# intel/oim

Hardware: AMD Instinct MI355X
Metric: 4KiB_randread_IOPS (higher is better)
Workload: dtype uint8

## Files before the change

### native/src/gpu.hip

```cpp

#include <hip/hip_runtime.h>
#include <pthread.h>
#include <sched.h>
#include <unistd.h>
#include <stdlib.h>

#include <algorithm>
#include <atomic>
#include <chrono>
#include <condition_variable>
#include <cstring>
#include <deque>
#include <functional>
#include <map>
#include <mutex>
#include <random>
#include <set>
#include <stdexcept>
#include <thread>
#include <utility>
#include <vector>

#include "gpu_internal.h"
#include "hipstore/engine.h"

namespace hipstore {


namespace {

constexpr uint32_t kTileBytes = 4096;
constexpr uint32_t kRingSlots = 1 << 16;
constexpr uint32_t kMaxBatchTiles = kRingSlots / 4;

struct BlockDesc {
  const uint8_t* src;
  uint8_t* dst;
  uint32_t bytes;
  uint32_t fill;
};
static_assert(sizeof(BlockDesc) == 24, "persistent engine reads 3 x u64");

__global__ __launch_bounds__(kWavesPerWg * 64) void k_copy_blocks(
    const BlockDesc* __restrict__ descs, uint32_t n) {
  __shared__ __attribute__((aligned(16))) uint8_t lds_raw[kWavesPerWg * kTileBytes];
  const uint32_t wave = threadIdx.x >> 6;
  const uint32_t lane = threadIdx.x & 63;
  const uint32_t idx = blockIdx.x * kWavesPerWg + wave;
  if (idx >= n) return;
  const BlockDesc d = descs[idx];
  float4* lds = reinterpret_cast<float4*>(lds_raw + wave * kTileBytes);
  const uint32_t n16 = d.bytes >> 4;
  if (d.src != nullptr) {
    const float4* __restrict__ src = reinterpret_cast<const float4*>(d.src);
#pragma unroll 4
    for (uint32_t i = lane; i < n16; i += 64) lds[i] = src[i];
  } else {
    const uint32_t b = d.fill & 0xFF;
    const uint32_t word = b | (b << 8) | (b << 16) | (b << 24);
    const float4 v = {__uint_as_float(word), __uint_as_float(word),
                      __uint_as_float(word), __uint_as_float(word)};
    for (uint32_t i = lane; i < n16; i += 64) lds[i] = v;
  }
  float4* __restrict__ dst = reinterpret_cast<float4*>(d.dst);
#pragma unroll 4
  for (uint32_t i = lane; i < n16; i += 64) dst[i] = lds[i];
}


__device__ __forceinline__ unsigned long long wave_bcast_u64(
    unsigned long long v) {
  int lo = __shfl(static_cast<int>(v & 0xFFFFFFFFu), 0);
  int hi = __shfl(static_cast<int>(v >> 32), 0);
  return (static_cast<unsigned long long>(static_cast<uint32_t>(hi)) << 32) |
         static_cast<uint32_t>(lo);
}

__device__ __forceinline__ unsigned long long claim_bounded(
    unsigned long long* counter, unsigned long long c,
    unsigned long long kt, uint32_t lane) {
  while (c < kt) {
    unsigned long long witnessed = 0;
    if (lane == 0) {
      witnessed = atomicCAS(counter, c, c + 1);
    }
    witnessed = wave_bcast_u64(witnessed);
    if (witnessed == c) return c;
    c = witnessed;
  }
  return ~0ull;
}

struct PersistentCtl {
  const BlockDesc* sq;
  volatile unsigned long long* sq_tail;
  volatile unsigned long long* cq;
  volatile uint32_t* stop;
  unsigned long long* claim_counter;
  unsigned long long* known_tail;
  uint32_t* exit_flag;
  uint32_t ring_mask;
  uint32_t idle_spins;
};

__global__ __launch_bounds__(64) void k_persistent_copy(PersistentCtl ctl) {
  __shared__ __attribute__((aligned(16))) uint8_t lds_raw[kTileBytes];
  const uint32_t lane = threadIdx.x & 63;
  float4* lds = reinterpret_cast<float4*>(lds_raw);

  if (blockIdx.x == 0) {
    if (lane != 0) return;
    unsigned long long known = __hip_atomic_load(
        ctl.known_tail, __ATOMIC_RELAXED, __HIP_MEMORY_SCOPE_AGENT);
    uint32_t spins = 0;
    while (true) {
      unsigned long long tail = __hip_atomic_load(
          const_cast<const unsigned long long*>(ctl.sq_tail),
          __ATOMIC_ACQUIRE, __HIP_MEMORY_SCOPE_SYSTEM);
      if (tail > known) {
        known = tail;
        __hip_atomic_store(ctl.known_tail, known, __ATOMIC_RELEASE,
                           __HIP_MEMORY_SCOPE_AGENT);
        spins = 0;
      }
      if (__hip_atomic_load(const_cast<const uint32_t*>(ctl.stop),
                            __ATOMIC_RELAXED,
                            __HIP_MEMORY_SCOPE_SYSTEM) != 0 ||
          ++spins > ctl.idle_spins) {
        __hip_atomic_store(ctl.exit_flag, 1u, __ATOMIC_RELEASE,
                           __HIP_MEMORY_SCOPE_AGENT);
        return;
      }
      __builtin_amdgcn_s_sleep(8);
    }
  }

  while (true) {
    const unsigned long long kt = __hip_atomic_load(
        ctl.known_tail, __ATOMIC_RELAXED, __HIP_MEMORY_SCOPE_AGENT);
    const unsigned long long c = __hip_atomic_load(
        ctl.claim_counter, __ATOMIC_RELAXED, __HIP_MEMORY_SCOPE_AGENT);
    const unsigned long long claim =
        claim_bounded(ctl.claim_counter, c, kt, lane);
    if (claim == ~0ull) {
      if (__hip_atomic_load(ctl.exit_flag, __ATOMIC_RELAXED,
                            __HIP_MEMORY_SCOPE_AGENT) != 0) {
        return;
      }
      __builtin_amdgcn_s_sleep(16);
      continue;
    }
    const volatile unsigned long long* vd =
        reinterpret_cast<const volatile unsigned long long*>(
            &ctl.sq[claim & ctl.ring_mask]);
    const unsigned long long w0 = vd[0];
    const unsigned long long w1 = vd[1];
    const unsigned long long w2 = vd[2];
    BlockDesc d;
    d.src = reinterpret_cast<const uint8_t*>(w0);
    d.dst = reinterpret_cast<uint8_t*>(w1);
    d.bytes = static_cast<uint32_t>(w2 & 0xFFFFFFFFu);
    d.fill = static_cast<uint32_t>(w2 >> 32);
    const uint32_t n8 = d.bytes >> 3;
    unsigned long long* lds64 = reinterpret_cast<unsigned long long*>(lds);
    if (d.src != nullptr) {
      const unsigned long long* __restrict__ src =
          reinterpret_cast<const unsigned long long*>(d.src);
#pragma unroll 4
      for (uint32_t i = lane; i < n8; i += 64) {
        lds64[i] = __hip_atomic_load(src + i, __ATOMIC_RELAXED,
                                     __HIP_MEMORY_SCOPE_AGENT);
      }
    } else {
      const uint32_t b = d.fill & 0xFF;
      const uint32_t word = b | (b << 8) | (b << 16) | (b << 24);
      const unsigned long long v =
          word | (static_cast<unsigned long long>(word) << 32);
      for (uint32_t i = lane; i < n8; i += 64) lds64[i] = v;
    }
    unsigned long long* __restrict__ dst =
        reinterpret_cast<unsigned long long*>(d.dst);
#pragma unroll 4
    for (uint32_t i = lane; i < n8; i += 64) dst[i] = lds64[i];
    if (lane == 0) {
      __hip_atomic_store(&ctl.cq[claim & ctl.ring_mask], claim + 1,
                         __ATOMIC_RELEASE, __HIP_MEMORY_SCOPE_SYSTEM);
    }
  }
}

__global__ void k_init_ctl(unsigned long long* dst, unsigned long long a,
                           unsigned long long b, unsigned long long c) {
  if (threadIdx.x == 0) {
    dst[0] = a;
    dst[1] = b;
    dst[2] = c;
  }
}

std::atomic<uint64_t> g_pers_launches{0};
std::atomic<uint64_t> g_pers_relaunches{0};
std::atomic<uint64_t> g_pers_stall_queries{0};


struct SharedSlot {
  const BlockDesc* sq;
  volatile unsigned long long* sq_tail;
  volatile unsigned long long* cq;
  unsigned long long claim;
  unsigned long long known_tail;
  unsigned long long ring_mask_active;
};
static_assert(sizeof(SharedSlot) == 48, "8-byte atom layout");

constexpr uint32_t kSharedSlots = 64;

struct SharedCtl {
  SharedSlot* slots;
  volatile uint32_t* stop;
  uint32_t* exit_flag;
  uint32_t idle_spins;
};

__device__ __forceinline__ unsigned long long slot_ld(
    SharedSlot* slot, int word) {
  return __hip_atomic_load(
      reinterpret_cast<unsigned long long*>(slot) + word, __ATOMIC_RELAXED,
      __HIP_MEMORY_SCOPE_AGENT);
}

__device__ __forceinline__ void slot_st(SharedSlot* slot, int word,
                                        unsigned long long value) {
  __hip_atomic_store(reinterpret_cast<unsigned long long*>(slot) + word,
                     value, __ATOMIC_RELEASE, __HIP_MEMORY_SCOPE_AGENT);
}

__global__ __launch_bounds__(64) void k_shared_service(SharedCtl ctl) {
  __shared__ __attribute__((aligned(16))) uint8_t lds_raw[kTileBytes];
  const uint32_t lane = threadIdx.x & 63;
  float4* lds = reinterpret_cast<float4*>(lds_raw);

  if (blockIdx.x == 0) {
    SharedSlot* slot = &ctl.slots[lane];
    unsigned long long known = 0;
    uint32_t spins = 0;
    while (true) {
      bool advanced = false;
      if (slot_ld(slot, 5) >> 32) {
        volatile unsigned long long* tail_ptr =
            reinterpret_cast<volatile unsigned long long*>(slot_ld(slot, 1));
        const unsigned long long tail = __hip_atomic_load(
            const_cast<const unsigned long long*>(tail_ptr),
            __ATOMIC_ACQUIRE, __HIP_MEMORY_SCOPE_SYSTEM);
        if (tail > known) {
          known = tail;
          slot_st(slot, 4, known);
          advanced = true;
        }
      } else {
        known = 0;
      }
      const bool stop_now =
          lane == 0 &&
          __hip_atomic_load(const_cast<const uint32_t*>(ctl.stop),
                            __ATOMIC_RELAXED,
                            __HIP_MEMORY_SCOPE_SYSTEM) != 0;
      if (__any(advanced)) spins = 0;
      if (__any(stop_now) || ++spins > ctl.idle_spins) {
        if (lane == 0) {
          __hip_atomic_store(ctl.exit_flag, 1u, __ATOMIC_RELEASE,
                             __HIP_MEMORY_SCOPE_AGENT);
        }
        return;
      }
      __builtin_amdgcn_s_sleep(8);
    }
  }

  const uint32_t start = blockIdx.x;
  while (true) {
    bool progress = false;
    for (uint32_t i = 0; i < kSharedSlots; ++i) {
      SharedSlot* slot = &ctl.slots[(start + i) % kSharedSlots];
      const unsigned long long ma = slot_ld(slot, 5);
      if (!(ma >> 32)) continue;
      const uint32_t ring_mask = static_cast<uint32_t>(ma);
      const unsigned long long kt = slot_ld(slot, 4);
      const unsigned long long c = slot_ld(slot, 3);
      const unsigned long long claim =
          claim_bounded(&slot->claim, c, kt, lane);
      if (claim == ~0ull) continue;
      const BlockDesc* sq = reinterpret_cast<const BlockDesc*>(slot_ld(slot, 0));
      const volatile unsigned long long* vd =
          reinterpret_cast<const volatile unsigned long long*>(
              &sq[claim & ring_mask]);
      const unsigned long long w0 = vd[0];
      const unsigned long long w1 = vd[1];
      const unsigned long long w2 = vd[2];
      const uint8_t* src = reinterpret_cast<const uint8_t*>(w0);
      uint8_t* dst = reinterpret_cast<uint8_t*>(w1);
      const uint32_t bytes = static_cast<uint32_t>(w2 & 0xFFFFFFFFu);
      const uint32_t n8 = bytes >> 3;
      unsigned long long* lds64 =
          reinterpret_cast<unsigned long long*>(lds);
      if (src != nullptr) {
        const unsigned long long* __restrict__ s8 =
            reinterpret_cast<const unsigned long long*>(src);
#pragma unroll 4
        for (uint32_t k = lane; k < n8; k += 64) {
          lds64[k] = __hip_atomic_load(s8 + k, __ATOMIC_RELAXED,
                                       __HIP_MEMORY_SCOPE_AGENT);
        }
      } else {
        const uint32_t b = static_cast<uint32_t>(w2 >> 32) & 0xFF;
        const uint32_t word = b | (b << 8) | (b << 16) | (b << 24);
        const unsigned long long v =
            word | (static_cast<unsigned long long>(word) << 32);
        for (uint32_t k = lane; k < n8; k += 64) lds64[k] = v;
      }
      unsigned long long* __restrict__ d8 =
          reinterpret_cast<unsigned long long*>(dst);
#pragma unroll 4
      for (uint32_t k = lane; k < n8; k += 64) d8[k] = lds64[k];
      if (lane == 0) {
        volatile unsigned long long* cq =
            reinterpret_cast<volatile unsigned long long*>(slot_ld(slot, 2));
        __hip_atomic_store(&cq[claim & ring_mask], claim + 1,
                           __ATOMIC_RELEASE, __HIP_MEMORY_SCOPE_SYSTEM);
      }
      progress = true;
    }
    if (!progress) {
      if (__hip_atomic_load(ctl.exit_flag, __ATOMIC_RELAXED,
                            __HIP_MEMORY_SCOPE_AGENT) != 0) {
        return;
      }
      __builtin_amdgcn_s_sleep(16);
    }
  }
}


struct ProbeCtl {
  volatile unsigned long long* sq_tail;
  volatile unsigned long long* hb_host;
  volatile unsigned long long* cq;
  unsigned long long* hb_dev;
  unsigned long long* relay;
  unsigned long long* rmw_counter;
  uint32_t use_atomics;
  uint32_t do_rmw;
  uint32_t do_fence;
  uint32_t max_spins;
};

__global__ __launch_bounds__(64) void k_probe(ProbeCtl ctl) {
  __shared__ __attribute__((aligned(16))) uint8_t lds_raw[kTileBytes];
  const uint32_t lane = threadIdx.x & 63;
  (void)lds_raw;
  if (lane != 0) return;
  if (blockIdx.x != 0) {
    for (uint32_t i = 0; i < ctl.max_spins; ++i) {
      if (ctl.do_rmw) {
        (void)__hip_atomic_fetch_add(ctl.rmw_counter, 1ull,
                                     __ATOMIC_RELAXED,
                                     __HIP_MEMORY_SCOPE_AGENT);
      }
      unsigned long long v =
          ctl.use_atomics
              ? __hip_atomic_load(ctl.relay, __ATOMIC_RELAXED,
                                  __HIP_MEMORY_SCOPE_AGENT)
              : *reinterpret_cast<volatile unsigned long long*>(ctl.relay);
      if (v != 0) {
        __hip_atomic_store(&ctl.cq[1], v, __ATOMIC_RELEASE,
                           __HIP_MEMORY_SCOPE_SYSTEM);
        return;
      }
      __builtin_amdgcn_s_sleep(8);
    }
    return;
  }
  for (uint32_t i = 0; i < ctl.max_spins; ++i) {
    if ((i & 1023) == 0) {
      const unsigned long long beat = i + 1;
      __hip_atomic_store(ctl.hb_dev, beat, __ATOMIC_RELAXED,
                         __HIP_MEMORY_SCOPE_AGENT);
      if (ctl.use_atomics) {
        __hip_atomic_store(ctl.hb_host, beat, __ATOMIC_RELAXED,
                           __HIP_MEMORY_SCOPE_SYSTEM);
      } else {
        *ctl.hb_host = beat;
      }
    }
    unsigned long long tail =
        ctl.use_atomics
            ? __hip_atomic_load(
                  const_cast<const unsigned long long*>(ctl.sq_tail),
                  __ATOMIC_ACQUIRE, __HIP_MEMORY_SCOPE_SYSTEM)
            : *ctl.sq_tail;
    if (tail != 0) {
      __hip_atomic_store(ctl.relay, tail, __ATOMIC_RELEASE,
                         __HIP_MEMORY_SCOPE_AGENT);
      if (ctl.do_fence) __threadfence_system();
      __hip_atomic_store(&ctl.cq[0], tail, __ATOMIC_RELEASE,
                         __HIP_MEMORY_SCOPE_SYSTEM);
      return;
    }
    __builtin_amdgcn_s_sleep(8);
  }
}

int g_device_count = -1;

struct HwQueueEnvInit {
  HwQueueEnvInit() {
    if (getenv("HIPSTORE_NO_HWQ_INIT") == nullptr) {
      setenv("GPU_MAX_HW_QUEUES", "24", 0);
    }
  }
};
HwQueueEnvInit g_hw_queue_env_init;

int device_count_cached() {
  static std::once_flag once;
  std::call_once(once, [] {
    int n = 0;
    if (hipGetDeviceCount(&n) != hipSuccess) n = 0;
    g_device_count = n;
  });
  return g_device_count;
}

double env_seconds(const char* name, double fallback) {
  const char* env = getenv(name);
  if (env == nullptr) return fallback;
  const double v = atof(env);
  return v > 0 ? v : fallback;
}

double sync_io_timeout_s() {
  static const double s = env_seconds("HIPSTORE_SYNC_TIMEOUT_S", 30.0);
  return s;
}

double teardown_timeout_s() {
  static const double s = env_seconds("HIPSTORE_TEARDOWN_TIMEOUT_S", 10.0);
  return s;
}

bool stream_drain(hipStream_t stream, double seconds) {
  const auto deadline = std::chrono::steady_clock::now() +
                        std::chrono::duration<double>(seconds);
  while (true) {
    if (hipStreamQuery(stream) != hipErrorNotReady) return true;
    if (std::chrono::steady_clock::now() > deadline) return false;
    std::this_thread::sleep_for(std::chrono::microseconds(200));
  }
}

void dump_engine_stats(const char* why) {
  fprintf(stderr,
          "[hipstore] %s: persistent-engine stats: launches=%llu "
          "relaunches=%llu stall_queries=%llu\n",
          why,
          static_cast<unsigned long long>(g_pers_launches.load()),
          static_cast<unsigned long long>(g_pers_relaunches.load()),
          static_cast<unsigned long long>(g_pers_stall_queries.load()));
}

}

uint64_t persistent_stat(int which) {
  switch (which) {
    case 0: return g_pers_launches.load();
    case 1: return g_pers_relaunches.load();
    case 2: return g_pers_stall_queries.load();
    default: return 0;
  }
}

bool gpu_available() { return device_count_cached() > 0; }
int gpu_device_count() { return device_count_cached(); }
// ... 234 lines not shown
    if (status != kIoOk) {
      immediate_.emplace_back(std::move(req.on_complete), status);
      return;
    }
    if (req.op == IoOp::kFlush) {
      flushes_.push_back({tail_, std::move(req.on_complete)});
      return;
    }
    pending_.push_back(std::move(req));
    drain_pending();
  }

  int poll() override {
    int completed = 0;
    if (!immediate_.empty()) {
      auto batch = std::move(immediate_);
      immediate_.clear();
      for (auto& [cb, status] : batch) {
        if (cb) cb(status);
        ++completed;
      }
    }
    const uint64_t retired_from = completed_;
    while (completed_ < tail_) {
      unsigned long long seq = __atomic_load_n(
          const_cast<const unsigned long long*>(&cq_[completed_ % kRing]),
          __ATOMIC_ACQUIRE);
      if (seq != completed_ + 1) break;
      IoState* state = desc_io_[completed_ % kRing];
      desc_io_[completed_ % kRing] = nullptr;
      ++completed_;
      if (state != nullptr && --state->remaining == 0) {
        if (state->cb) state->cb(state->status);
        delete state;
        ++completed;
      }
    }
    if (completed_ != retired_from) on_retired(completed_);
    while (!flushes_.empty() && flushes_.front().first <= completed_) {
      if (flushes_.front().second) flushes_.front().second(kIoOk);
      flushes_.pop_front();
      ++completed;
    }
    drain_pending();
    if (completed > 0) last_progress_ = std::chrono::steady_clock::now();
    if (completed_ < tail_) {
      const auto now = std::chrono::steady_clock::now();
      if (now - last_progress_ > std::chrono::milliseconds(1)) {
        on_stall();
        last_progress_ = now;
      }
    }
    return completed;
  }

 protected:
  explicit ServiceRingChannel(uint8_t* base) : base_(base) {}

  ~ServiceRingChannel() override = default;

  virtual void on_retired(uint64_t ) {}
  virtual void on_stall() = 0;

  void alloc_rings() {
    HIP_CHECK(hipHostMalloc(reinterpret_cast<void**>(&sq_),
                            kRing * sizeof(BlockDesc), hipHostMallocMapped));
    void* p_tail = nullptr;
    void* p_cq = nullptr;
    HIP_CHECK(hipHostMalloc(&p_tail, 8, hipHostMallocMapped));
    HIP_CHECK(hipHostMalloc(&p_cq, kRing * 8, hipHostMallocMapped));
    sq_tail_ = static_cast<volatile unsigned long long*>(p_tail);
    cq_ = static_cast<volatile unsigned long long*>(p_cq);
    *sq_tail_ = 0;
    memset(const_cast<unsigned long long*>(cq_), 0, kRing * 8);
    desc_io_.resize(kRing, nullptr);
  }

  void free_rings() {
    (void)hipHostFree(sq_);
    (void)hipHostFree(const_cast<unsigned long long*>(sq_tail_));
    (void)hipHostFree(const_cast<unsigned long long*>(cq_));
  }

  void delete_unfired() {
    std::set<IoState*> leftovers(desc_io_.begin(), desc_io_.end());
    for (IoState* state : leftovers) delete state;
  }

  BlockDesc* sq_ = nullptr;
  volatile unsigned long long* sq_tail_ = nullptr;
  volatile unsigned long long* cq_ = nullptr;
  uint64_t tail_ = 0;
  uint64_t completed_ = 0;
  std::chrono::steady_clock::time_point last_progress_{};

 private:
  struct IoState {
    IoCompletion cb;
    uint32_t remaining;
    int status;
  };

  bool has_capacity(uint32_t tiles) const {
    return tail_ - completed_ + tiles <= kRing;
  }

  void drain_pending() {
    while (!pending_.empty()) {
      IoRequest& req = pending_.front();
      const uint32_t tiles = tile_count(req.length);
      if (!has_capacity(tiles)) return;
      auto* state = new IoState{std::move(req.on_complete), tiles, kIoOk};
      uint64_t done = 0;
      uint64_t t = tail_;
      while (done < req.length) {
        const uint32_t bytes = static_cast<uint32_t>(
            std::min<uint64_t>(kTileBytes, req.length - done));
        fill_desc(sq_[t % kRing], req, base_, done, bytes);
        desc_io_[t % kRing] = state;
        ++t;
        done += bytes;
      }
      tail_ = t;
      __atomic_store_n(const_cast<unsigned long long*>(sq_tail_), tail_,
                       __ATOMIC_RELEASE);
      pending_.pop_front();
    }
  }

  uint8_t* base_;
  std::vector<IoState*> desc_io_;
  std::deque<IoRequest> pending_;
  std::deque<std::pair<uint64_t, IoCompletion>> flushes_;
  std::vector<std::pair<IoCompletion, int>> immediate_;
};

inline std::atomic<int> g_per_queue_channels[64];
inline int per_queue_channel_cap() {
  static const int cap = [] {
    const char* env = getenv("HIPSTORE_PERQ_CAP");
    return env ? atoi(env) : 18;
  }();
  return cap;
}

inline bool fallback_is_shared() {
  static const bool shared = [] {
    const char* env = getenv("HIPSTORE_FALLBACK");
    return env == nullptr || strcmp(env, "batched") != 0;
  }();
  return shared;
}

class HbmPersistentChannel : public ServiceRingChannel {
 public:
  static constexpr uint32_t kIdleSpins = 500000;

  static uint32_t workers() {
    static uint32_t w = [] {
      const char* env = getenv("HIPSTORE_PERSISTENT_WORKERS");
      int v = env ? atoi(env) : 16;
      return static_cast<uint32_t>(std::min(std::max(v, 1), 64));
    }();
    return w;
  }

  HbmPersistentChannel(int device, uint8_t* base)
      : ServiceRingChannel(base), device_(device) {
    HIP_CHECK(hipSetDevice(device));
    HIP_CHECK(hipStreamCreateWithFlags(&stream_, hipStreamNonBlocking));
    alloc_rings();
    void* p_stop = nullptr;
    HIP_CHECK(hipHostMalloc(&p_stop, 4, hipHostMallocMapped));
    stop_ = static_cast<volatile uint32_t*>(p_stop);
    *stop_ = 0;
    HIP_CHECK(hipMalloc(reinterpret_cast<void**>(&claim_ctr_), 24));
    HIP_CHECK(hipMemset(claim_ctr_, 0, 24));
    HIP_CHECK(hipStreamSynchronize(nullptr));
    launch();
  }

  ~HbmPersistentChannel() override {
    g_per_queue_channels[device_].fetch_sub(1, std::memory_order_relaxed);
    __atomic_store_n(const_cast<uint32_t*>(stop_), 1u, __ATOMIC_RELEASE);
    if (!stream_drain(stream_, teardown_timeout_s())) {
      dump_engine_stats(
          "persistent-channel teardown timeout; leaking rings");
      return;
    }
    free_rings();
    (void)hipHostFree(const_cast<uint32_t*>(stop_));
    (void)hipFree(claim_ctr_);
    (void)hipStreamDestroy(stream_);
    delete_unfired();
  }

  const char* kind_name() const override { return "persistent"; }

 private:
  void on_stall() override {
    g_pers_stall_queries.fetch_add(1, std::memory_order_relaxed);
    if (hipStreamQuery(stream_) == hipSuccess) {
      g_pers_relaunches.fetch_add(1, std::memory_order_relaxed);
      launch();
    }
    debug_dump_state();
  }

  void launch() {
    g_pers_launches.fetch_add(1, std::memory_order_relaxed);
    (void)hipSetDevice(device_);
    static const bool use_memcpy = [] {
      const char* env = getenv("HIPSTORE_LAUNCH_INIT");
      return env != nullptr && strcmp(env, "memcpy") == 0;
    }();
    if (use_memcpy) {
      const unsigned long long init[3] = {completed_, completed_, 0};
      HIP_CHECK(hipMemcpyAsync(claim_ctr_, init, 24, hipMemcpyHostToDevice,
                               stream_));
    } else {
      hipLaunchKernelGGL(k_init_ctl, dim3(1), dim3(1), 0, stream_,
                         claim_ctr_, completed_, completed_, 0ull);
    }
    PersistentCtl ctl;
    ctl.sq = device_view(sq_);
    ctl.sq_tail = device_view(const_cast<unsigned long long*>(sq_tail_));
    ctl.cq = device_view(const_cast<unsigned long long*>(cq_));
    ctl.stop = device_view(const_cast<uint32_t*>(stop_));
    ctl.claim_counter = claim_ctr_;
    ctl.known_tail = claim_ctr_ + 1;
    ctl.exit_flag = reinterpret_cast<uint32_t*>(claim_ctr_ + 2);
    ctl.ring_mask = kRing - 1;
    ctl.idle_spins = kIdleSpins;
    hipLaunchKernelGGL(k_persistent_copy, dim3(workers() + 1), dim3(64), 0,
                       stream_, ctl);
    const hipError_t err = hipGetLastError();
    if (err != hipSuccess) {
      fprintf(stderr, "[hipstore] persistent service launch failed: %s\n",
              hipGetErrorString(err));
    }
    last_progress_ = std::chrono::steady_clock::now();
  }

  void debug_dump_state() {
    static const bool debug = getenv("HIPSTORE_DEBUG") != nullptr;
    if (!debug) return;
    const auto now = std::chrono::steady_clock::now();
    if (now - dbg_last_ < std::chrono::seconds(1)) return;
    dbg_last_ = now;
    if (dbg_stream_ == nullptr) {
      if (hipStreamCreateWithFlags(&dbg_stream_, hipStreamNonBlocking) !=
          hipSuccess) {
        return;
      }
    }
    unsigned long long words[3] = {0, 0, 0};
    (void)hipMemcpyAsync(words, claim_ctr_, 24, hipMemcpyDeviceToHost,
                         dbg_stream_);
    (void)hipStreamSynchronize(dbg_stream_);
    fprintf(stderr,
            "[hipstore-dbg] perq tail=%llu done=%llu sq_tail=%llu "
            "dev_claim=%llu dev_known=%llu dev_exit=%llu busy=%d\n",
            static_cast<unsigned long long>(tail_),
            static_cast<unsigned long long>(completed_), *sq_tail_,
            words[0], words[1], words[2],
            hipStreamQuery(stream_) == hipErrorNotReady);
  }

  std::chrono::steady_clock::time_point dbg_last_{};
  hipStream_t dbg_stream_ = nullptr;

  int device_;
  hipStream_t stream_ = nullptr;
  volatile uint32_t* stop_ = nullptr;
  unsigned long long* claim_ctr_ = nullptr;
};

class SharedService {
 public:
  static constexpr uint32_t kIdleSpins = 500000;

  static std::shared_ptr<SharedService>& instance(int device) {
    static std::mutex mutex;
    static std::map<int, std::shared_ptr<SharedService>> services;
    std::lock_guard<std::mutex> lock(mutex);
    auto& service = services[device];
    if (!service) service = std::make_shared<SharedService>(device);
    return service;
  }

  explicit SharedService(int device) : device_(device) {
    dbg("svc:setdev");
    HIP_CHECK(hipSetDevice(device));
    HIP_CHECK(hipStreamCreateWithFlags(&stream_, hipStreamNonBlocking));
    HIP_CHECK(hipStreamCreateWithFlags(&config_stream_, hipStreamNonBlocking));
    dbg("svc:malloc");
    HIP_CHECK(hipMalloc(reinterpret_cast<void**>(&slots_dev_),
                        kSharedSlots * sizeof(SharedSlot) + 8));
    dbg("svc:memset");
    HIP_CHECK(hipMemset(slots_dev_, 0, kSharedSlots * sizeof(SharedSlot) + 8));
    dbg("svc:nullsync");
    HIP_CHECK(hipStreamSynchronize(nullptr));
    dbg("svc:hostmalloc");
    exit_flag_dev_ = reinterpret_cast<uint32_t*>(slots_dev_ + kSharedSlots);
    void* p_stop = nullptr;
    HIP_CHECK(hipHostMalloc(&p_stop, 4, hipHostMallocMapped));
    stop_ = static_cast<volatile uint32_t*>(p_stop);
    *stop_ = 0;
    memset(mirror_, 0, sizeof(mirror_));
    memset(used_, 0, sizeof(used_));
    memset(prefix_, 0, sizeof(prefix_));
    HIP_CHECK(hipMemsetAsync(exit_flag_dev_, 0, 4, stream_));
    HIP_CHECK(hipMemsetAsync(exit_flag_dev_, 0, 4, config_stream_));
    HIP_CHECK(hipStreamSynchronize(stream_));
    HIP_CHECK(hipStreamSynchronize(config_stream_));
    dbg("svc:ctor-done");
  }

  static void dbg(const char* what) {
    if (getenv("HIPSTORE_DEBUG") != nullptr) {
      fprintf(stderr, "[hipstore-dbg] %s\n", what);
    }
  }


  int attach(const BlockDesc* sq_dev, unsigned long long* tail_dev,
             unsigned long long* cq_dev, uint32_t ring_mask) {
    std::lock_guard<std::mutex> lock(mutex_);
    for (uint32_t i = 0; i < kSharedSlots; ++i) {
      if (used_[i]) continue;
      used_[i] = true;
      prefix_[i] = 0;
      SharedSlot& m = mirror_[i];
      m.sq = sq_dev;
      m.sq_tail = tail_dev;
      m.cq = cq_dev;
      m.claim = 0;
      m.known_tail = 0;
      m.ring_mask_active = ring_mask;
      (void)hipSetDevice(device_);
      dbg("attach:copy");
      HIP_CHECK(hipMemcpyAsync(&slots_dev_[i], &m, 40, hipMemcpyHostToDevice,
                               config_stream_));
      m.ring_mask_active = ring_mask | (1ull << 32);
      HIP_CHECK(hipMemcpyAsync(
          reinterpret_cast<unsigned long long*>(&slots_dev_[i]) + 5,
          &m.ring_mask_active, 8, hipMemcpyHostToDevice, config_stream_));
      dbg("attach:sync");
      HIP_CHECK(hipStreamSynchronize(config_stream_));
      dbg("attach:launch");
      ensure_running_locked(true);
      dbg("attach:done");
      return static_cast<int>(i);
    }
    throw std::runtime_error("shared service: no free ring slots (64 max)");
  }

  void detach(int slot) {
    std::lock_guard<std::mutex> lock(mutex_);
    (void)hipSetDevice(device_);
    mirror_[slot].ring_mask_active &= 0xFFFFFFFFull;
    (void)hipMemcpyAsync(
        reinterpret_cast<unsigned long long*>(&slots_dev_[slot]) + 5,
        &mirror_[slot].ring_mask_active, 8, hipMemcpyHostToDevice,
        config_stream_);
    (void)hipStreamSynchronize(config_stream_);
    used_[slot] = false;
  }

  void update_prefix(int slot, uint64_t completed) {
    prefix_[slot] = completed;
  }

  void ensure_running() {
    std::lock_guard<std::mutex> lock(mutex_);
    ensure_running_locked(false);
  }

 private:
  void ensure_running_locked(bool force_check) {
    const auto now = std::chrono::steady_clock::now();
    if (!force_check && now - last_check_ < std::chrono::milliseconds(1)) {
      return;
    }
    last_check_ = now;
    if (hipStreamQuery(stream_) != hipSuccess) return;
    (void)hipSetDevice(device_);
    for (uint32_t i = 0; i < kSharedSlots; ++i) {
      if (!used_[i]) continue;
      mirror_[i].claim = prefix_[i];
      mirror_[i].known_tail = prefix_[i];
    }
    HIP_CHECK(hipMemcpyAsync(slots_dev_, mirror_,
                             kSharedSlots * sizeof(SharedSlot),
                             hipMemcpyHostToDevice, stream_));
    HIP_CHECK(hipMemsetAsync(exit_flag_dev_, 0, 4, stream_));
    SharedCtl ctl;
    ctl.slots = slots_dev_;
    ctl.stop = device_view(const_cast<uint32_t*>(stop_));
    ctl.exit_flag = exit_flag_dev_;
    ctl.idle_spins = kIdleSpins;
    const char* env = getenv("HIPSTORE_SHARED_WORKERS");
    int workers = env ? atoi(env) : 48;
    workers = std::min(std::max(workers, 1), 255);
    hipLaunchKernelGGL(k_shared_service, dim3(workers + 1), dim3(64), 0,
                       stream_, ctl);
    if (getenv("HIPSTORE_DEBUG") != nullptr) {
      hipError_t launch_err = hipGetLastError();
      hipError_t query = hipStreamQuery(stream_);
      fprintf(stderr, "[hipstore-dbg] svc:launched err=%d query=%d\n",
              static_cast<int>(launch_err), static_cast<int>(query));
    }
    g_pers_launches.fetch_add(1, std::memory_order_relaxed);
  }

 public:
  void debug_read_slot(int slot, unsigned long long out[3]) {
    std::lock_guard<std::mutex> lock(mutex_);
    (void)hipSetDevice(device_);
    (void)hipMemcpyAsync(out,
                         reinterpret_cast<unsigned long long*>(
                             &slots_dev_[slot]) + 3,
                         24, hipMemcpyDeviceToHost, config_stream_);
    (void)hipStreamSynchronize(config_stream_);
  }

 private:

  int device_;
  hipStream_t stream_ = nullptr;
  hipStream_t config_stream_ = nullptr;
  SharedSlot* slots_dev_ = nullptr;
  uint32_t* exit_flag_dev_ = nullptr;
  volatile uint32_t* stop_ = nullptr;
  std::mutex mutex_;
  SharedSlot mirror_[kSharedSlots];
  bool used_[kSharedSlots];
  uint64_t prefix_[kSharedSlots];
  std::chrono::steady_clock::time_point last_check_{};
};

class HbmSharedChannel : public ServiceRingChannel {
 public:
  HbmSharedChannel(int device, uint8_t* base) : ServiceRingChannel(base) {
    SharedService::dbg("chan:instance");
    service_ = SharedService::instance(device);
    SharedService::dbg("chan:hostmalloc");
    HIP_CHECK(hipSetDevice(device));
    alloc_rings();
    SharedService::dbg("chan:attach");
    slot_ = service_->attach(
        device_view(sq_), device_view(const_cast<unsigned long long*>(sq_tail_)),
        device_view(const_cast<unsigned long long*>(cq_)), kRing - 1);
  }

  ~HbmSharedChannel() override {
    const auto deadline = std::chrono::steady_clock::now() +
                          std::chrono::duration<double>(teardown_timeout_s());
    while (completed_ < tail_ &&
           std::chrono::steady_clock::now() < deadline) {
      poll();
    }
    service_->detach(slot_);
    delete_unfired();
    if (completed_ < tail_) {
      dump_engine_stats("shared-channel teardown timeout; leaking rings");
      return;
    }
    free_rings();
  }

  const char* kind_name() const override { return "shared"; }

  int poll() override {
    static const bool debug_env = getenv("HIPSTORE_DEBUG") != nullptr;
    if (debug_env) {
      const auto now = std::chrono::steady_clock::now();
      if (now - dbg_last_ > std::chrono::seconds(2)) {
        dbg_last_ = now;
        unsigned long long st[3] = {0, 0, 0};
        service_->debug_read_slot(slot_, st);
        fprintf(stderr,
                "[hipstore-dbg] slot=%d tail=%llu done=%llu sqtail=%llu "
                "dev_claim=%llu dev_kt=%llu dev_ma=%llx\n",
                slot_, static_cast<unsigned long long>(tail_),
                static_cast<unsigned long long>(completed_), *sq_tail_,
                st[0], st[1], st[2]);
      }
    }
    return ServiceRingChannel::poll();
  }

 private:
  void on_retired(uint64_t completed) override {
    service_->update_prefix(slot_, completed);
  }

  void on_stall() override { service_->ensure_running(); }

  std::shared_ptr<SharedService> service_;
  std::chrono::steady_clock::time_point dbg_last_{};
  int slot_ = -1;
};

class HbmBdev : public Bdev {
 public:
  HbmBdev(const std::string& name, uint64_t block_size, uint64_t num_blocks,
          int device, bool persistent)
      : Bdev(name, "Malloc disk", block_size, num_blocks),
        device_(device),
        persistent_(persistent) {
    if (persistent_) {
      const char* env = getenv("HIPSTORE_SHARED");
      shared_ = env != nullptr && atoi(env) != 0;
    }
    HIP_CHECK(hipSetDevice(device));
    HIP_CHECK(hipMalloc(reinterpret_cast<void**>(&base_), size_bytes()));
    HIP_CHECK(hipMemset(base_, 0, size_bytes()));
    HIP_CHECK(hipStreamSynchronize(nullptr));
  }

  ~HbmBdev() override {
    (void)hipSetDevice(device_);
    (void)hipFree(base_);
  }

  int device() const { return device_; }
  void* device_base() override { return base_; }
  int gpu_device() const override { return device_; }

  int resize(uint64_t new_num_blocks) override {
    std::lock_guard<std::mutex> lock(resize_mutex_);
    if (live_channels_->load(std::memory_order_acquire) != 0) {
      return kIoFailed;
    }
    const uint64_t old_bytes = size_bytes();
    const uint64_t new_bytes = new_num_blocks * block_size();
    if (new_bytes == old_bytes) return kIoOk;
    HIP_CHECK(hipSetDevice(device_));
    uint8_t* new_base = nullptr;
    if (hipMalloc(reinterpret_cast<void**>(&new_base), new_bytes) !=
        hipSuccess) {
      return kIoFailed;
    }
    hipStream_t stream = nullptr;
    HIP_CHECK(hipStreamCreateWithFlags(&stream, hipStreamNonBlocking));
    const uint64_t keep = std::min(old_bytes, new_bytes);
    if (new_bytes > old_bytes) {
      HIP_CHECK(hipMemsetAsync(new_base + keep, 0, new_bytes - keep, stream));
    }
    const uint64_t n16 = keep / 16;
    const uint32_t grid = static_cast<uint32_t>(
        std::min<uint64_t>(2048, (n16 + 255) / 256));
    hipLaunchKernelGGL(k_copy_range, dim3(grid), dim3(256), 0, stream,
// ... 667 lines not shown
  if (failed) throw std::runtime_error("perf session: I/O failures");
  result.iops = result.io_count / elapsed;
  result.throughput_mbps =
      result.io_count * static_cast<double>(im.io_size) / elapsed / 1e6;
  total.fill_result(&result);
  return result;
}

std::map<std::string, long long> persistent_probe(int device, int flags) {
  std::map<std::string, long long> r;
  const bool use_atomics = flags & 1;
  const bool pre_memcpy = flags & 2;
  const bool do_rmw = flags & 4;
  const bool big_grid = flags & 8;
  const bool do_fence = flags & 16;
  r["flags"] = flags;
  HIP_CHECK(hipSetDevice(device));
  hipStream_t stream = nullptr;
  hipStream_t util = nullptr;
  HIP_CHECK(hipStreamCreateWithFlags(&stream, hipStreamNonBlocking));
  HIP_CHECK(hipStreamCreateWithFlags(&util, hipStreamNonBlocking));
  void* p_tail = nullptr;
  void* p_hb = nullptr;
  void* p_cq = nullptr;
  HIP_CHECK(hipHostMalloc(&p_tail, 8, hipHostMallocMapped));
  HIP_CHECK(hipHostMalloc(&p_hb, 8, hipHostMallocMapped));
  HIP_CHECK(hipHostMalloc(&p_cq, 16, hipHostMallocMapped));
  auto* tail = static_cast<volatile unsigned long long*>(p_tail);
  auto* hb = static_cast<volatile unsigned long long*>(p_hb);
  auto* cq = static_cast<volatile unsigned long long*>(p_cq);
  *tail = 0;
  *hb = 0;
  cq[0] = 0;
  cq[1] = 0;
  unsigned long long* dev_words = nullptr;
  HIP_CHECK(hipMalloc(reinterpret_cast<void**>(&dev_words), 24));
  HIP_CHECK(hipMemset(dev_words, 0, 24));
  HIP_CHECK(hipStreamSynchronize(nullptr));
  ProbeCtl ctl;
  ctl.sq_tail = device_view(const_cast<unsigned long long*>(tail));
  ctl.hb_host = device_view(const_cast<unsigned long long*>(hb));
  ctl.cq = device_view(const_cast<unsigned long long*>(cq));
  ctl.hb_dev = dev_words;
  ctl.relay = dev_words + 1;
  ctl.rmw_counter = dev_words + 2;
  ctl.use_atomics = use_atomics ? 1 : 0;
  ctl.do_rmw = do_rmw ? 1 : 0;
  ctl.do_fence = do_fence ? 1 : 0;
  ctl.max_spins = 4u << 20;
  if (pre_memcpy) {
    const unsigned long long init[3] = {0, 0, 0};
    HIP_CHECK(hipMemcpyAsync(dev_words, init, 24, hipMemcpyHostToDevice,
                             stream));
  }
  hipLaunchKernelGGL(k_probe, dim3(big_grid ? 17 : 2), dim3(64), 0, stream,
                     ctl);
  r["launch_err"] = static_cast<long long>(hipGetLastError());
  using clock = std::chrono::steady_clock;
  const auto t0 = clock::now();
  std::this_thread::sleep_for(std::chrono::milliseconds(250));
  r["hb_host_early"] =
      static_cast<long long>(__atomic_load_n(hb, __ATOMIC_ACQUIRE));
  unsigned long long hb_dev_early = 0;
  (void)hipMemcpyAsync(&hb_dev_early, dev_words, 8, hipMemcpyDeviceToHost,
                       util);
  (void)hipStreamSynchronize(util);
  r["hb_dev_early"] = static_cast<long long>(hb_dev_early);
  __atomic_store_n(tail, 1ull, __ATOMIC_RELEASE);
  r["cq0_ms"] = -1;
  r["cq1_ms"] = -1;
  while (clock::now() - t0 < std::chrono::seconds(5)) {
    if (r["cq0_ms"] < 0 && __atomic_load_n(&cq[0], __ATOMIC_ACQUIRE) != 0) {
      r["cq0_ms"] = std::chrono::duration_cast<std::chrono::milliseconds>(
                        clock::now() - t0).count();
    }
    if (r["cq1_ms"] < 0 && __atomic_load_n(&cq[1], __ATOMIC_ACQUIRE) != 0) {
      r["cq1_ms"] = std::chrono::duration_cast<std::chrono::milliseconds>(
                        clock::now() - t0).count();
    }
    if (r["cq0_ms"] >= 0 && r["cq1_ms"] >= 0) break;
    std::this_thread::sleep_for(std::chrono::milliseconds(2));
  }
  r["hb_host_final"] =
      static_cast<long long>(__atomic_load_n(hb, __ATOMIC_ACQUIRE));
  unsigned long long dev_final[3] = {0, 0, 0};
  (void)hipMemcpyAsync(dev_final, dev_words, 24, hipMemcpyDeviceToHost,
                       util);
  (void)hipStreamSynchronize(util);
  r["hb_dev_final"] = static_cast<long long>(dev_final[0]);
  r["relay_final"] = static_cast<long long>(dev_final[1]);
  r["rmw_final"] = static_cast<long long>(dev_final[2]);
  const bool drained = stream_drain(stream, 10.0);
  r["stream_drained"] = drained;
  if (drained) {
    (void)hipHostFree(p_tail);
    (void)hipHostFree(p_hb);
    (void)hipHostFree(p_cq);
    (void)hipFree(dev_words);
    (void)hipStreamDestroy(stream);
  }
  (void)hipStreamDestroy(util);
  return r;
}


std::map<std::string, long long> persistent_kernel_probe(int device,
                                                         int variant) {
  constexpr uint32_t kProbeRing = 32768;
  std::map<std::string, long long> r;
  r["variant"] = variant;
  HIP_CHECK(hipSetDevice(device));
  hipStream_t stream = nullptr;
  hipStream_t util = nullptr;
  HIP_CHECK(hipStreamCreateWithFlags(&stream, hipStreamNonBlocking));
  HIP_CHECK(hipStreamCreateWithFlags(&util, hipStreamNonBlocking));
  BlockDesc* sq = nullptr;
  HIP_CHECK(hipHostMalloc(reinterpret_cast<void**>(&sq),
                          kProbeRing * sizeof(BlockDesc),
                          hipHostMallocMapped));
  void* p_tail = nullptr;
  void* p_cq = nullptr;
  void* p_stop = nullptr;
  void* p_buf = nullptr;
  HIP_CHECK(hipHostMalloc(&p_tail, 8, hipHostMallocMapped));
  HIP_CHECK(hipHostMalloc(&p_cq, kProbeRing * 8, hipHostMallocMapped));
  HIP_CHECK(hipHostMalloc(&p_stop, 4, hipHostMallocMapped));
  HIP_CHECK(hipHostMalloc(&p_buf, 8192, hipHostMallocMapped));
  auto* tail = static_cast<volatile unsigned long long*>(p_tail);
  auto* cq = static_cast<volatile unsigned long long*>(p_cq);
  auto* stop = static_cast<volatile uint32_t*>(p_stop);
  auto* buf = static_cast<uint8_t*>(p_buf);
  *tail = 0;
  *stop = 0;
  memset(const_cast<unsigned long long*>(cq), 0, kProbeRing * 8);
  memset(buf, 0x5A, 4096);
  memset(buf + 4096, 0, 4096);
  uint8_t* hbm = nullptr;
  HIP_CHECK(hipMalloc(reinterpret_cast<void**>(&hbm), 8192));
  HIP_CHECK(hipMemset(hbm, 0xA7, 8192));
  unsigned long long* claim_ctr = nullptr;
  HIP_CHECK(hipMalloc(reinterpret_cast<void**>(&claim_ctr), 24));
  HIP_CHECK(hipMemset(claim_ctr, 0, 24));
  HIP_CHECK(hipStreamSynchronize(nullptr));
  PersistentCtl ctl;
  ctl.sq = device_view(sq);
  ctl.sq_tail = device_view(const_cast<unsigned long long*>(tail));
  ctl.cq = device_view(const_cast<unsigned long long*>(cq));
  ctl.stop = device_view(const_cast<uint32_t*>(stop));
  ctl.claim_counter = claim_ctr;
  ctl.known_tail = claim_ctr + 1;
  ctl.exit_flag = reinterpret_cast<uint32_t*>(claim_ctr + 2);
  ctl.ring_mask = kProbeRing - 1;
  ctl.idle_spins = 500000;
  hipLaunchKernelGGL(k_persistent_copy, dim3(17), dim3(64), 0, stream, ctl);
  r["launch_err"] = static_cast<long long>(hipGetLastError());
  uint8_t* buf_dev = device_view(buf);
  BlockDesc& d = sq[0];
  switch (variant) {
    case 0:
      d.src = buf_dev;
      d.dst = buf_dev + 4096;
      d.bytes = 64;
      break;
    case 1:
      d.src = buf_dev;
      d.dst = hbm;
      d.bytes = 4096;
      break;
    default:
      d.src = hbm;
      d.dst = buf_dev + 4096;
      d.bytes = 4096;
      break;
  }
  d.fill = 0;
  __atomic_store_n(tail, 1ull, __ATOMIC_RELEASE);
  using clock = std::chrono::steady_clock;
  const auto t0 = clock::now();
  r["cq_ms"] = -1;
  while (clock::now() - t0 < std::chrono::seconds(4)) {
    if (__atomic_load_n(&cq[0], __ATOMIC_ACQUIRE) == 1) {
      r["cq_ms"] = std::chrono::duration_cast<std::chrono::milliseconds>(
                       clock::now() - t0).count();
      break;
    }
    std::this_thread::sleep_for(std::chrono::milliseconds(2));
  }
  unsigned long long words[3] = {0, 0, 0};
  (void)hipMemcpyAsync(words, claim_ctr, 24, hipMemcpyDeviceToHost, util);
  (void)hipStreamSynchronize(util);
  r["dev_claim"] = static_cast<long long>(words[0]);
  r["dev_known"] = static_cast<long long>(words[1]);
  r["dev_exit"] = static_cast<long long>(words[2]);
  r["data_ok"] = variant == 0   ? memcmp(buf, buf + 4096, 64) == 0
                 : variant == 2 ? buf[4096] == 0xA7 && buf[8191] == 0xA7
                                : -1;
  __atomic_store_n(stop, 1u, __ATOMIC_RELEASE);
  const bool drained = stream_drain(stream, 8.0);
  r["stream_drained"] = drained;
  if (drained) {
    (void)hipHostFree(sq);
    (void)hipHostFree(p_tail);
    (void)hipHostFree(p_cq);
    (void)hipHostFree(p_stop);
    (void)hipHostFree(p_buf);
    (void)hipFree(hbm);
    (void)hipFree(claim_ctr);
    (void)hipStreamDestroy(stream);
  }
  (void)hipStreamDestroy(util);
  return r;
}


}
```

Measured before the change: 11.94 million.

## Claim runs of descriptors per wave and copy tiles via registers

Measured after the change: 12.74 million (median of 6 runs). 1.07x the previous value.

```diff
diff --git a/native/src/gpu.hip b/native/src/gpu.hip
--- a/native/src/gpu.hip
+++ b/native/src/gpu.hip
@@ -68,27 +68,112 @@
 }
 
 
-__device__ __forceinline__ unsigned long long wave_bcast_u64(
-    unsigned long long v) {
-  int lo = __shfl(static_cast<int>(v & 0xFFFFFFFFu), 0);
-  int hi = __shfl(static_cast<int>(v >> 32), 0);
+__device__ __forceinline__ unsigned long long wave_shfl_u64(
+    unsigned long long v, uint32_t src_lane) {
+  const int from = static_cast<int>(src_lane);
+  int lo = __shfl(static_cast<int>(v & 0xFFFFFFFFu), from);
+  int hi = __shfl(static_cast<int>(v >> 32), from);
   return (static_cast<unsigned long long>(static_cast<uint32_t>(hi)) << 32) |
          static_cast<uint32_t>(lo);
 }
 
-__device__ __forceinline__ unsigned long long claim_bounded(
+typedef __attribute__((address_space(1))) unsigned long long gu64;
+typedef const __attribute__((address_space(1))) unsigned long long cgu64;
+
+__device__ __forceinline__ gu64* as_global(const volatile void* p) {
+  return reinterpret_cast<gu64*>(reinterpret_cast<uintptr_t>(p));
+}
+
+constexpr uint32_t kMaxRunTiles = 8;
+
+__device__ __forceinline__ unsigned long long claim_run(
     unsigned long long* counter, unsigned long long c,
-    unsigned long long kt, uint32_t lane) {
+    unsigned long long kt, uint32_t workers, uint32_t batch, uint32_t lane,
+    uint32_t* n_out) {
   while (c < kt) {
+    const unsigned long long cap =
+        static_cast<unsigned long long>(batch) * workers;
+    const uint32_t backlog =
+        static_cast<uint32_t>(kt - c < cap ? kt - c : cap);
+    const uint32_t n = (backlog + workers - 1) / workers;
     unsigned long long witnessed = 0;
     if (lane == 0) {
-      witnessed = atomicCAS(counter, c, c + 1);
-    }
-    witnessed = wave_bcast_u64(witnessed);
-    if (witnessed == c) return c;
+      witnessed = atomicCAS(counter, c, c + n);
+    }
+    witnessed = wave_shfl_u64(witnessed, 0);
+    if (witnessed == c) {
+      *n_out = n;
+      return c;
+    }
     c = witnessed;
   }
   return ~0ull;
+}
+
+template <bool kFull>
+__device__ __forceinline__ void move_tile(
+    unsigned long long src_word, unsigned long long dst_word, uint32_t n8,
+    unsigned long long fill64, uint32_t lane) {
+  unsigned long long v[8];
+#pragma unroll
+  for (uint32_t k = 0; k < 8; ++k) v[k] = fill64;
+  if (src_word != 0) {
+    cgu64* src = reinterpret_cast<cgu64*>(src_word);
+#pragma unroll
+    for (uint32_t k = 0; k < 8; ++k) {
+      const uint32_t i = lane + 64 * k;
+      if (kFull || i < n8) {
+        v[k] = __hip_atomic_load(src + i, __ATOMIC_RELAXED,
+                                 __HIP_MEMORY_SCOPE_AGENT);
+      }
+    }
+  }
+  gu64* dst = reinterpret_cast<gu64*>(dst_word);
+#pragma unroll
+  for (uint32_t j = 0; j < 8; ++j) {
+    const uint32_t k = kFull ? j : 7 - j;
+    const uint32_t i = lane + 64 * k;
+    if (kFull || i < n8) {
+      __hip_atomic_store(dst + i, v[k], __ATOMIC_RELAXED,
+                         __HIP_MEMORY_SCOPE_SYSTEM);
+    }
+  }
+}
+
+__device__ __forceinline__ void serve_run(
+    const BlockDesc* sq, volatile unsigned long long* cq, uint32_t ring_mask,
+    unsigned long long claim, uint32_t n, uint32_t lane) {
+  static_assert(3 * kMaxRunTiles <= 64, "descriptor words of a run: one load");
+  static_assert(kTileBytes == 8 * 64 * 8, "8 x u64 per lane per tile");
+  const uint32_t my_tile = lane / 3;
+  const uint32_t my_word = lane - 3 * my_tile;
+  unsigned long long word = 0;
+  if (lane < 3 * n) {
+    cgu64* slot =
+        as_global(sq) + 3ull * ((claim + my_tile) & ring_mask) + my_word;
+    word = __hip_atomic_load(slot, __ATOMIC_RELAXED, __HIP_MEMORY_SCOPE_SYSTEM);
+  }
+  for (uint32_t t = 0; t < n; ++t) {
+    const unsigned long long w0 = wave_shfl_u64(word, 3 * t);
+    const unsigned long long w1 = wave_shfl_u64(word, 3 * t + 1);
+    const unsigned long long w2 = wave_shfl_u64(word, 3 * t + 2);
+    const uint32_t n8 = static_cast<uint32_t>(w2 & 0xFFFFFFFFu) >> 3;
+    const uint32_t b = static_cast<uint32_t>(w2 >> 32) & 0xFF;
+    const uint32_t fill32 = b | (b << 8) | (b << 16) | (b << 24);
+    const unsigned long long fill64 =
+        fill32 | (static_cast<unsigned long long>(fill32) << 32);
+    if (n8 == kTileBytes / 8) {
+      move_tile<true>(w0, w1, n8, fill64, lane);
+    } else {
+      move_tile<false>(w0, w1, n8, fill64, lane);
+    }
+  }
+  asm volatile("s_waitcnt vmcnt(0)" ::: "memory");
+  if (lane < n) {
+    const unsigned long long index = claim + lane;
+    __hip_atomic_store(as_global(&cq[index & ring_mask]), index + 1,
+                       __ATOMIC_RELAXED, __HIP_MEMORY_SCOPE_SYSTEM);
+  }
 }
 
 struct PersistentCtl {
@@ -101,12 +186,11 @@
   uint32_t* exit_flag;
   uint32_t ring_mask;
   uint32_t idle_spins;
+  uint32_t batch_tiles;
 };
 
 __global__ __launch_bounds__(64) void k_persistent_copy(PersistentCtl ctl) {
-  __shared__ __attribute__((aligned(16))) uint8_t lds_raw[kTileBytes];
   const uint32_t lane = threadIdx.x & 63;
-  float4* lds = reinterpret_cast<float4*>(lds_raw);
 
   if (blockIdx.x == 0) {
     if (lane != 0) return;
@@ -135,13 +219,15 @@
     }
   }
 
+  const uint32_t workers = gridDim.x - 1;
   while (true) {
     const unsigned long long kt = __hip_atomic_load(
         ctl.known_tail, __ATOMIC_RELAXED, __HIP_MEMORY_SCOPE_AGENT);
     const unsigned long long c = __hip_atomic_load(
         ctl.claim_counter, __ATOMIC_RELAXED, __HIP_MEMORY_SCOPE_AGENT);
-    const unsigned long long claim =
-        claim_bounded(ctl.claim_counter, c, kt, lane);
+    uint32_t n = 0;
+    const unsigned long long claim = claim_run(
+        ctl.claim_counter, c, kt, workers, ctl.batch_tiles, lane, &n);
     if (claim == ~0ull) {
       if (__hip_atomic_load(ctl.exit_flag, __ATOMIC_RELAXED,
                             __HIP_MEMORY_SCOPE_AGENT) != 0) {
@@ -150,42 +236,7 @@
       __builtin_amdgcn_s_sleep(16);
       continue;
     }
-    const volatile unsigned long long* vd =
-        reinterpret_cast<const volatile unsigned long long*>(
-            &ctl.sq[claim & ctl.ring_mask]);
-    const unsigned long long w0 = vd[0];
-    const unsigned long long w1 = vd[1];
-    const unsigned long long w2 = vd[2];
-    BlockDesc d;
-    d.src = reinterpret_cast<const uint8_t*>(w0);
-    d.dst = reinterpret_cast<uint8_t*>(w1);
-    d.bytes = static_cast<uint32_t>(w2 & 0xFFFFFFFFu);
-    d.fill = static_cast<uint32_t>(w2 >> 32);
-    const uint32_t n8 = d.bytes >> 3;
-    unsigned long long* lds64 = reinterpret_cast<unsigned long long*>(lds);
-    if (d.src != nullptr) {
-      const unsigned long long* __restrict__ src =
-          reinterpret_cast<const unsigned long long*>(d.src);
-#pragma unroll 4
-      for (uint32_t i = lane; i < n8; i += 64) {
-        lds64[i] = __hip_atomic_load(src + i, __ATOMIC_RELAXED,
-                                     __HIP_MEMORY_SCOPE_AGENT);
-      }
-    } else {
-      const uint32_t b = d.fill & 0xFF;
-      const uint32_t word = b | (b << 8) | (b << 16) | (b << 24);
-      const unsigned long long v =
-          word | (static_cast<unsigned long long>(word) << 32);
-      for (uint32_t i = lane; i < n8; i += 64) lds64[i] = v;
-    }
-    unsigned long long* __restrict__ dst =
-        reinterpret_cast<unsigned long long*>(d.dst);
-#pragma unroll 4
-    for (uint32_t i = lane; i < n8; i += 64) dst[i] = lds64[i];
-    if (lane == 0) {
-      __hip_atomic_store(&ctl.cq[claim & ctl.ring_mask], claim + 1,
-                         __ATOMIC_RELEASE, __HIP_MEMORY_SCOPE_SYSTEM);
-    }
+    serve_run(ctl.sq, ctl.cq, ctl.ring_mask, claim, n, lane);
   }
 }
 
@@ -220,6 +271,7 @@
   volatile uint32_t* stop;
   uint32_t* exit_flag;
   uint32_t idle_spins;
+  uint32_t batch_tiles;
 };
 
 __device__ __forceinline__ unsigned long long slot_ld(
@@ -236,9 +288,7 @@
 }
 
 __global__ __launch_bounds__(64) void k_shared_service(SharedCtl ctl) {
-  __shared__ __attribute__((aligned(16))) uint8_t lds_raw[kTileBytes];
   const uint32_t lane = threadIdx.x & 63;
-  float4* lds = reinterpret_cast<float4*>(lds_raw);
 
   if (blockIdx.x == 0) {
     SharedSlot* slot = &ctl.slots[lane];
@@ -278,6 +328,7 @@
   }
 
   const uint32_t start = blockIdx.x;
+  const uint32_t workers = gridDim.x - 1;
   while (true) {
     bool progress = false;
     for (uint32_t i = 0; i < kSharedSlots; ++i) {
@@ -287,47 +338,14 @@
       const uint32_t ring_mask = static_cast<uint32_t>(ma);
       const unsigned long long kt = slot_ld(slot, 4);
       const unsigned long long c = slot_ld(slot, 3);
-      const unsigned long long claim =
-          claim_bounded(&slot->claim, c, kt, lane);
+      uint32_t n = 0;
+      const unsigned long long claim = claim_run(
+          &slot->claim, c, kt, workers, ctl.batch_tiles, lane, &n);
       if (claim == ~0ull) continue;
       const BlockDesc* sq = reinterpret_cast<const BlockDesc*>(slot_ld(slot, 0));
-      const volatile unsigned long long* vd =
-          reinterpret_cast<const volatile unsigned long long*>(
-              &sq[claim & ring_mask]);
-      const unsigned long long w0 = vd[0];
-      const unsigned long long w1 = vd[1];
-      const unsigned long long w2 = vd[2];
-      const uint8_t* src = reinterpret_cast<const uint8_t*>(w0);
-      uint8_t* dst = reinterpret_cast<uint8_t*>(w1);
-      const uint32_t bytes = static_cast<uint32_t>(w2 & 0xFFFFFFFFu);
-      const uint32_t n8 = bytes >> 3;
-      unsigned long long* lds64 =
-          reinterpret_cast<unsigned long long*>(lds);
-      if (src != nullptr) {
-        const unsigned long long* __restrict__ s8 =
-            reinterpret_cast<const unsigned long long*>(src);
-#pragma unroll 4
-        for (uint32_t k = lane; k < n8; k += 64) {
-          lds64[k] = __hip_atomic_load(s8 + k, __ATOMIC_RELAXED,
-                                       __HIP_MEMORY_SCOPE_AGENT);
-        }
-      } else {
-        const uint32_t b = static_cast<uint32_t>(w2 >> 32) & 0xFF;
-        const uint32_t word = b | (b << 8) | (b << 16) | (b << 24);
-        const unsigned long long v =
-            word | (static_cast<unsigned long long>(word) << 32);
-        for (uint32_t k = lane; k < n8; k += 64) lds64[k] = v;
-      }
-      unsigned long long* __restrict__ d8 =
-          reinterpret_cast<unsigned long long*>(dst);
-#pragma unroll 4
-      for (uint32_t k = lane; k < n8; k += 64) d8[k] = lds64[k];
-      if (lane == 0) {
-        volatile unsigned long long* cq =
-            reinterpret_cast<volatile unsigned long long*>(slot_ld(slot, 2));
-        __hip_atomic_store(&cq[claim & ring_mask], claim + 1,
-                           __ATOMIC_RELEASE, __HIP_MEMORY_SCOPE_SYSTEM);
-      }
+      volatile unsigned long long* cq =
+          reinterpret_cast<volatile unsigned long long*>(slot_ld(slot, 2));
+      serve_run(sq, cq, ring_mask, claim, n, lane);
       progress = true;
     }
     if (!progress) {
@@ -868,21 +886,28 @@
   return shared;
 }
 
+inline uint32_t batch_tiles_env() {
+  const char* env = getenv("HIPSTORE_BATCH_TILES");
+  const int v = env ? atoi(env) : 2;
+  return static_cast<uint32_t>(
+      std::min(std::max(v, 1), static_cast<int>(kMaxRunTiles)));
+}
+
 class HbmPersistentChannel : public ServiceRingChannel {
  public:
   static constexpr uint32_t kIdleSpins = 500000;
 
-  static uint32_t workers() {
-    static uint32_t w = [] {
-      const char* env = getenv("HIPSTORE_PERSISTENT_WORKERS");
-      int v = env ? atoi(env) : 16;
-      return static_cast<uint32_t>(std::min(std::max(v, 1), 64));
-    }();
-    return w;
+  static uint32_t workers_env() {
+    const char* env = getenv("HIPSTORE_PERSISTENT_WORKERS");
+    int v = env ? atoi(env) : 16;
+    return static_cast<uint32_t>(std::min(std::max(v, 1), 64));
   }
 
   HbmPersistentChannel(int device, uint8_t* base)
-      : ServiceRingChannel(base), device_(device) {
+      : ServiceRingChannel(base),
+        device_(device),
+        workers_(workers_env()),
+        batch_tiles_(batch_tiles_env()) {
     HIP_CHECK(hipSetDevice(device));
     HIP_CHECK(hipStreamCreateWithFlags(&stream_, hipStreamNonBlocking));
     alloc_rings();
@@ -948,7 +973,8 @@
     ctl.exit_flag = reinterpret_cast<uint32_t*>(claim_ctr_ + 2);
     ctl.ring_mask = kRing - 1;
     ctl.idle_spins = kIdleSpins;
-    hipLaunchKernelGGL(k_persistent_copy, dim3(workers() + 1), dim3(64), 0,
+    ctl.batch_tiles = batch_tiles_;
+    hipLaunchKernelGGL(k_persistent_copy, dim3(workers_ + 1), dim3(64), 0,
                        stream_, ctl);
     const hipError_t err = hipGetLastError();
     if (err != hipSuccess) {
@@ -987,6 +1013,8 @@
   hipStream_t dbg_stream_ = nullptr;
 
   int device_;
+  const uint32_t workers_;
+  const uint32_t batch_tiles_;
   hipStream_t stream_ = nullptr;
   volatile uint32_t* stop_ = nullptr;
   unsigned long long* claim_ctr_ = nullptr;
@@ -1116,6 +1144,7 @@
     ctl.stop = device_view(const_cast<uint32_t*>(stop_));
     ctl.exit_flag = exit_flag_dev_;
     ctl.idle_spins = kIdleSpins;
+    ctl.batch_tiles = batch_tiles_env();
     const char* env = getenv("HIPSTORE_SHARED_WORKERS");
     int workers = env ? atoi(env) : 48;
     workers = std::min(std::max(workers, 1), 255);
@@ -2089,6 +2118,7 @@
   ctl.exit_flag = reinterpret_cast<uint32_t*>(claim_ctr + 2);
   ctl.ring_mask = kProbeRing - 1;
   ctl.idle_spins = 500000;
+  ctl.batch_tiles = 1;
   hipLaunchKernelGGL(k_persistent_copy, dim3(17), dim3(64), 0, stream, ctl);
   r["launch_err"] = static_cast<long long>(hipGetLastError());
   uint8_t* buf_dev = device_view(buf);
```
